# zuds-survey/zuds-pipeline

Hardware: AMD Instinct MI355X
Metric: Mpix/s resample->coadd->subtract, 3072x3072 frames (higher is better)
Workload: dtype f32; 1 GPU; configs[1]+[2]: 32x 3072x3072 TPV frames/GPU, mesh background + weight rescale + Lanczos-3 resample + WEIGHTED coadd (+ AND mask coadd, int16 masks); then 1 science frame/GPU: align ref, hotpants 3x3 regions x 10x10 stamps, r=10, ko=4, subtract; frames_per_gpu=32, size=3072, mask_dtype=int16, combine=WEIGHTED, subtract=True

## Files before the change

zuds-pipeline_amd/csrc/hotpants.hip:

```cpp
#include "hp_dev.h"
#include <sched.h>
#include "chol_diag.h"

__global__ void k_hp_valid(const float* __restrict__ sci, const float* __restrict__ ref,
                           const uint8_t* __restrict__ bpm, int64_t n, float il, float iu,
                           float tl, float tu, uint8_t* __restrict__ bad,
                           const double* __restrict__ lim, double nsig) {
    int64_t p = (int64_t)blockIdx.x * blockDim.x + threadIdx.x;
    if (lim) {
        il = (float)(lim[0] - nsig * lim[1]);
        tl = (float)(lim[3] - nsig * lim[4]);
    }
    if (p >= n) return;
    float s = sci[p], t = ref[p];
    bool ok = (s == s) && (t == t) && fabsf(s) < 3e38f && fabsf(t) < 3e38f;
    ok = ok && s >= il && s <= iu && t >= tl && t <= tu;
    if (bpm) ok = ok && bpm[p] == 0;
    bad[p] = ok ? 0 : 1;
}

#define HP_ROWMAX 16384
__global__ __launch_bounds__(256) void k_hp_rowany(const uint8_t* __restrict__ in, int nx, int ny, int hw,
                                                   uint8_t* __restrict__ out) {
    extern __shared__ int ra_pre[];
    __shared__ int wsum[4];
    const int y = blockIdx.x, tid = threadIdx.x;
    const uint8_t* row = in + (size_t)y * nx;
    const int per = (nx + 255) / 256;
    const int x0 = tid * per, x1 = min(x0 + per, nx);
    int loc = 0;
    for (int x = x0; x < x1; ++x) loc += row[x] ? 1 : 0;
    int inc = loc;
    const int lane = tid & 63, wave = tid >> 6;
#pragma unroll
    for (int o = 1; o < 64; o <<= 1) {
        const int t = __shfl_up(inc, o);
        if (lane >= o) inc += t;
    }
    if (lane == 63) wsum[wave] = inc;
    __syncthreads();
    int base = inc - loc;
    for (int w = 0; w < wave; ++w) base += wsum[w];
    if (tid == 0) ra_pre[0] = 0;
    int run = base;
    for (int x = x0; x < x1; ++x) { run += row[x] ? 1 : 0; ra_pre[x + 1] = run; }
    __syncthreads();
    for (int x = tid; x < nx; x += 256) {
        const int a = max(x - hw, 0), b = min(x + hw, nx - 1);
        out[(size_t)y * nx + x] = (ra_pre[b + 1] - ra_pre[a]) > 0;
    }
}

__global__ __launch_bounds__(256) void k_hp_valid_rows(const float* __restrict__ sci, const float* __restrict__ ref,
                                                       const uint8_t* __restrict__ bpm, int nx, int ny, float il, float iu,
                                                       float tl, float tu, const double* __restrict__ lim, double nsig,
                                                       int hw1, int hw2, uint8_t* __restrict__ bad,
                                                       uint8_t* __restrict__ out1, uint8_t* __restrict__ out2) {
    extern __shared__ int ra_pre[];
    __shared__ int wsum[HP_ROWMAX / 64], wtot[4];
    if (lim) {
        il = (float)(lim[0] - nsig * lim[1]);
        tl = (float)(lim[3] - nsig * lim[4]);
    }
    const int y = blockIdx.x, tid = threadIdx.x;
    const size_t r0 = (size_t)y * nx;
    const int lane = tid & 63, wave = tid >> 6;
    const int nch = (nx + 255) / 256;
    for (int c = 0; c < nch; ++c) {
        const int x = 256 * c + tid;
        bool b = false;
        if (x < nx) {
            const float s = sci[r0 + x], t = ref[r0 + x];
            bool ok = (s == s) && (t == t) && fabsf(s) < 3e38f && fabsf(t) < 3e38f;
            ok = ok && s >= il && s <= iu && t >= tl && t <= tu;
            if (bpm) ok = ok && bpm[r0 + x] == 0;
            b = !ok;
            bad[r0 + x] = b ? 1 : 0;
        }
        const unsigned long long m = __ballot(b);
        if (x < nx) ra_pre[x + 1] = __popcll(m & ((2ull << lane) - 1ull));
        if (lane == 0) wsum[4 * c + wave] = __popcll(m);
    }
    if (tid == 0) ra_pre[0] = 0;
    __syncthreads();
    {
        const int v = tid < 4 * nch ? wsum[tid] : 0;
        int inc = v;
#pragma unroll
        for (int o = 1; o < 64; o <<= 1) {
            const int t = __shfl_up(inc, o);
            if (lane >= o) inc += t;
        }
        if (lane == 63) wtot[wave] = inc;
        __syncthreads();
        int off = inc - v;
        for (int w = 0; w < wave; ++w) off += wtot[w];
        if (tid < 4 * nch) wsum[tid] = off;
    }
    __syncthreads();
    for (int c = 0; c < nch; ++c) {
        const int x = 256 * c + tid;
        if (x < nx) ra_pre[x + 1] += wsum[4 * c + wave];
    }
    __syncthreads();
    for (int x = tid; x < nx; x += 256) {
        const int a1 = max(x - hw1, 0), b1 = min(x + hw1, nx - 1);
        const int a2 = max(x - hw2, 0), b2 = min(x + hw2, nx - 1);
        out1[r0 + x] = (ra_pre[b1 + 1] - ra_pre[a1]) > 0;
        out2[r0 + x] = (ra_pre[b2 + 1] - ra_pre[a2]) > 0;
    }
}
// ... 387 lines not shown
        for (int k = threadIdx.x; k < nzero; k += 256) zero[(size_t)reg * nzero + k] = 0u;
    const int c1 = blockIdx.y * 16 + (threadIdx.x >> 4), c2 = blockIdx.x * 16 + (threadIdx.x & 15);
    if (blockIdx.x > blockIdx.y) return;
    if (c1 >= P.nunk || c2 >= P.nunk) return;
    int n1, p1, n2, p2;
    col_decode(P, c1, &n1, &p1);
    col_decode(P, c2, &n2, &p2);
    double acc = 0.0, racc = 0.0;
    const bool do_rhs = (c2 == 0);
    bool any = false;
    const int* list = chg + P.ncell + reg * (P.ncellr + 1);
    const int ncand = (sign == 0) ? P.ncellr : list[0];
    for (int s0 = 0; s0 < ncand; s0 += 8) {
        double g[8], gr[8], w1[8], w2[8];
        bool on[8];
#pragma unroll
        for (int u = 0; u < 8; ++u) {
            const int s = s0 + u;
            on[u] = false;
            g[u] = gr[u] = 0.0;
            w1[u] = w2[u] = 1.0;
            if (s < ncand) {
                const int cell = (sign == 0) ? reg * P.ncellr + s : list[1 + s];
                on[u] = !(active[cell] < 0 && sign >= 0);
                if (on[u]) {
                    const double* Gc = G + (size_t)cell * HP_MAXX * HP_MAXX;
                    const double* ph = phi + (size_t)cell * P.nkp;
                    if (p1 >= 0) w1[u] = ph[p1];
                    if (p2 >= 0) w2[u] = ph[p2];
                    g[u] = Gc[n1 * HP_MAXX + n2];
                    if (do_rhs) gr[u] = Gc[n1 * HP_MAXX + P.nE];
                }
            }
        }
#pragma unroll
        for (int u = 0; u < 8; ++u)
            if (on[u]) {
                any = true;
                acc += w1[u] * w2[u] * g[u];
                if (do_rhs) racc += w1[u] * gr[u];
            }
    }
    const size_t ia = (size_t)reg * (size_t)(P.nunk + 1) * P.nunk + (size_t)c1 * P.nunk + c2;
    if (sign == 0) {
        if (c2 <= c1) A[ia] = acc;
        if (do_rhs) rhs[(size_t)reg * P.nunk + c1] = racc;
    } else if (any) {
        if (c2 <= c1) A[ia] += sign * acc;
        if (do_rhs) rhs[(size_t)reg * P.nunk + c1] += sign * racc;
    }
}

#define BB_CH 128
static __device__ __forceinline__ void hp_build_blk_body(const int reg, const int pair, const hp_plan& P, const double* __restrict__ G,
                                                      const double* __restrict__ phi,
                                                      const int* __restrict__ active,
                                                      const int* __restrict__ chg, int sign,
                                                      double* __restrict__ A,
                                                      double* __restrict__ rhs, const int* __restrict__ guard,
                                                      unsigned* __restrict__ zero, int nzero,
                                                      const double* __restrict__ Gold,
                                                      const double* __restrict__ phiold,
                                                      const int* __restrict__ need) {
    if (guard && *guard == 0) return;
    int n1 = (int)((sqrtf(8.f * (float)pair + 1.f) - 1.f) * 0.5f);
    while (n1 * (n1 + 1) / 2 > pair) --n1;
    while ((n1 + 1) * (n1 + 2) / 2 <= pair) ++n1;
    const int n2 = pair - n1 * (n1 + 1) / 2;
    if (zero && n1 == 0 && n2 == 0)
        for (int k = threadIdx.x; k < nzero; k += 256) zero[(size_t)reg * nzero + k] = 0u;
    const int p1 = threadIdx.x >> 4, p2 = threadIdx.x & 15;
    const bool k1 = n1 >= 1 && n1 < P.nc, k2 = n2 >= 1 && n2 < P.nc;
    const int nk = (P.nc - 1) * P.nkp;
    const int c1 = n1 == 0 ? 0 : (k1 ? 1 + (n1 - 1) * P.nkp + p1 : 1 + nk + (n1 - P.nc));
    const int c2 = n2 == 0 ? 0 : (k2 ? 1 + (n2 - 1) * P.nkp + p2 : 1 + nk + (n2 - P.nc));
    const bool live = p1 < (k1 ? P.nkp : 1) && p2 < (k2 ? P.nkp : 1) && c2 <= c1;
    const bool do_rhs = (c2 == 0);
    const int* list = chg + P.ncell + reg * (P.ncellr + 1);
    const int ncand = (sign == 0) ? P.ncellr : list[0];
    __shared__ double gs[BB_CH], grs[BB_CH], phs[BB_CH * 16];
    __shared__ int ons[BB_CH];
    const int tid = threadIdx.x;
    const size_t ia = (size_t)reg * (size_t)(P.nunk + 1) * P.nunk + (size_t)c1 * P.nunk + c2;
    double av = 0.0, rv = 0.0;
    bool touched = false;
    const int npass = sign == 2 ? 2 : 1;
    for (int pass = 0; pass < npass; ++pass) {
        const int sg = sign == 2 ? (pass == 0 ? -1 : 1) : sign;
        double acc = 0.0, racc = 0.0;
        bool any = false;
        for (int s0 = 0; s0 < ncand; s0 += BB_CH) {
            const int nch = min(BB_CH, ncand - s0);
            __syncthreads();
            if (tid < nch) {
                const int cell = (sg == 0) ? reg * P.ncellr + s0 + tid : list[1 + s0 + tid];
                const int on = !(active[cell] < 0 && sg >= 0);
                const bool was = sign == 2 && pass == 0 && need[cell];
                const double* Gc = (was ? Gold : G) + (size_t)cell * HP_MAXX * HP_MAXX;
                ons[tid] = on;
                gs[tid] = on ? Gc[n1 * HP_MAXX + n2] : 0.0;
                grs[tid] = (on && n2 == 0) ? Gc[n1 * HP_MAXX + P.nE] : 0.0;
            }
            for (int e = tid; e < nch * P.nkp; e += 256) {
                const int k = e / P.nkp, pp = e - k * P.nkp;
                const int cell = (sg == 0) ? reg * P.ncellr + s0 + k : list[1 + s0 + k];
                const bool was = sign == 2 && pass == 0 && need[cell];
                phs[k * 16 + pp] = (was ? phiold : phi)[(size_t)cell * P.nkp + pp];
            }
            __syncthreads();
            if (live) {
                for (int k = 0; k < nch; ++k) {
                    if (!ons[k]) continue;
                    any = true;
                    const double w1 = k1 ? phs[k * 16 + p1] : 1.0, w2 = k2 ? phs[k * 16 + p2] : 1.0;
                    acc += w1 * w2 * gs[k];
                    if (do_rhs) racc += w1 * grs[k];
                }
            }
        }
        if (!live) continue;
        if (sg == 0) {
            A[ia] = acc;
            if (do_rhs) rhs[(size_t)reg * P.nunk + c1] = racc;
        } else if (any) {
            if (!touched) {
                av = A[ia];
                if (do_rhs) rv = rhs[(size_t)reg * P.nunk + c1];
                touched = true;
            }
            av += (double)sg * acc;
            if (do_rhs) rv += (double)sg * racc;
        }
    }
    if (live && touched) {
        A[ia] = av;
        if (do_rhs) rhs[(size_t)reg * P.nunk + c1] = rv;
    }
}

#define BM_CH 128
static __device__ __forceinline__ void hp_build_mfma_body(const hp_plan& P, const double* __restrict__ G,
                                                       const double* __restrict__ phi, const int* __restrict__ active,
                                                       double* __restrict__ A, double* __restrict__ rhs,
                                                       unsigned* __restrict__ zero, int nzero) {
    typedef double bm_double4 __attribute__((ext_vector_type(4)));
    __shared__ double phs[BM_CH][16];
    __shared__ double gw[4][2][BM_CH];
    const int reg = blockIdx.y, tid = threadIdx.x, wave = tid >> 6, lane = tid & 63, li = lane & 15, lk = lane >> 4;
    if (zero && blockIdx.x == 0)
        for (int k = tid; k < nzero; k += 256) zero[(size_t)reg * nzero + k] = 0u;
    const int npair = P.nE * (P.nE + 1) / 2;
    const int pair = blockIdx.x * 4 + wave;
    const bool have = pair < npair;
    int n1 = 0, n2 = 0;
    if (have) {
        n1 = (int)((sqrtf(8.f * (float)pair + 1.f) - 1.f) * 0.5f);
        while (n1 * (n1 + 1) / 2 > pair) --n1;
        while ((n1 + 1) * (n1 + 2) / 2 <= pair) ++n1;
        n2 = pair - n1 * (n1 + 1) / 2;
    }
    const bool k1 = n1 >= 1 && n1 < P.nc, k2 = n2 >= 1 && n2 < P.nc;
    const int nk = (P.nc - 1) * P.nkp;
    const int b1 = n1 == 0 ? 0 : (k1 ? 1 + (n1 - 1) * P.nkp : 1 + nk + (n1 - P.nc));
    const int b2 = n2 == 0 ? 0 : (k2 ? 1 + (n2 - 1) * P.nkp : 1 + nk + (n2 - P.nc));
    const int np1 = k1 ? P.nkp : 1, np2 = k2 ? P.nkp : 1;
    bm_double4 c4 = {0.0, 0.0, 0.0, 0.0};
    for (int s0 = 0; s0 < P.ncellr; s0 += BM_CH) {
        const int nch = min(BM_CH, P.ncellr - s0);
        __syncthreads();
        for (int e = tid; e < BM_CH * 16; e += 256) {
            const int k = e >> 4, pp = e & 15;
            double v = 0.0;
            if (k < nch && pp < P.nkp) {
                const int cell = reg * P.ncellr + s0 + k;
                if (active[cell] >= 0) v = phi[(size_t)cell * P.nkp + pp];
            }
            phs[k][pp] = v;
        }
        for (int k = lane; k < BM_CH; k += 64) {
            double g = 0.0, gr = 0.0;
            if (have && k < nch) {
                const int cell = reg * P.ncellr + s0 + k;
                if (active[cell] >= 0) {
                    const double* Gc = G + (size_t)cell * HP_MAXX * HP_MAXX;
                    g = Gc[n1 * HP_MAXX + n2];
                    if (n2 == 0) gr = Gc[n1 * HP_MAXX + P.nE];
                }
            }
            gw[wave][0][k] = g;
            gw[wave][1][k] = gr;
// ... 1428 lines not shown
    used = wave_sum_d(used);
    if (lane == 0) {
        nrej[reg] = (int)cnt;
        if (cnt > 0) atomicAdd(round_flag, (int)cnt);
        if (tmo && tmo[reg]) atomicOr(round_flag, HP_RFLAG_TMO);
        stats[reg * 2 + 0] = used > 0 ? msum / used : 0.0;
        stats[reg * 2 + 1] = used;
    }
    int* list = chg + P.ncell + reg * (P.ncellr + 1);
    int base = 0;
#pragma unroll
    for (int u = 0; u < 4; ++u) {
        const unsigned long long bm = chm[u];
        if (bm >> lane & 1ull)
            list[1 + base + __popcll(bm & ((1ull << lane) - 1ull))] = reg * P.ncellr + lane + 64 * u;
        base += __popcll(bm);
    }
    if (lane == 0) list[0] = base;
}

__global__ void k_hp_init_active(const hp_plan P, const int2* __restrict__ centres,
                                 int* __restrict__ active, int* __restrict__ need,
                                 int* __restrict__ ntotal) {
    int cell = blockIdx.x * blockDim.x + threadIdx.x;
    if (cell >= P.ncell) return;
    bool has = centres[cell * P.nss].x >= 0;
    active[cell] = has ? 0 : -1;
    need[cell] = has ? 1 : 0;
    if (has) atomicAdd(&ntotal[cell / P.ncellr], 1);
}

__global__ __launch_bounds__(256) void k_hp_gram(const hp_plan P, const double* __restrict__ X,
                                                 const int* __restrict__ need, const int* __restrict__ active,
                                                 double* __restrict__ Gp, const int* __restrict__ guard,
                                                 const int* __restrict__ list) {
    hp_gram_body(P, X, need, active, Gp, guard, list);
}
__global__ __launch_bounds__(256) void k_hp_gram_b(const hp_plan P, const hp_job* __restrict__ jobs, int round) {
    const hp_job& J = jobs[blockIdx.z];
    hp_gram_body(P, J.X, J.need, J.active, J.Gp, HPJ_GUARD(J, round), round > 1 ? J.needlist : nullptr);
}

__global__ __launch_bounds__(GS_THREADS) void k_hp_gram_sum(const double* __restrict__ Gp, const int* __restrict__ need,
                                                     const int* __restrict__ active, double* __restrict__ G,
                                                     const int* __restrict__ guard, double* __restrict__ Gold,
                                                     const int* __restrict__ list) {
    hp_gram_sum_body(Gp, need, active, G, guard, Gold, list);
}
__global__ __launch_bounds__(GS_THREADS) void k_hp_gram_sum_b(const hp_job* __restrict__ jobs, int round) {
    const hp_job& J = jobs[blockIdx.z];
    hp_gram_sum_body(J.Gp, J.need, J.active, J.G, HPJ_GUARD(J, round), J.Gold, round > 1 ? J.needlist : nullptr);
}

#define HBB_PAIRS 5
__global__ __launch_bounds__(256) void k_hp_build_blk(const hp_plan P, const double* __restrict__ G,
                                                      const double* __restrict__ phi, const int* __restrict__ active,
                                                      const int* __restrict__ chg, int sign, double* __restrict__ A,
                                                      double* __restrict__ rhs, const int* __restrict__ guard,
                                                      unsigned* __restrict__ zero = nullptr, int nzero = 0,
                                                      const double* __restrict__ Gold = nullptr,
                                                      const double* __restrict__ phiold = nullptr,
                                                      const int* __restrict__ need = nullptr) {
    if (guard && *guard == 0) return;
    const int reg = blockIdx.z;
    if (sign == 2 && chg[P.ncell + reg * (P.ncellr + 1)] == 0) {
        if (zero && blockIdx.x == 0)
            for (int k = threadIdx.x; k < nzero; k += 256) zero[(size_t)reg * nzero + k] = 0u;
        return;
    }
    const int npair = P.nE * (P.nE + 1) / 2;
#pragma unroll 1
    for (int pair = blockIdx.x * HBB_PAIRS; pair < min((int)(blockIdx.x + 1) * HBB_PAIRS, npair); ++pair)
        hp_build_blk_body(reg, pair, P, G, phi, active, chg, sign, A, rhs, guard, zero, nzero, Gold, phiold, need);
}
__global__ __launch_bounds__(256) void k_hp_build_blk_b(const hp_plan P, const hp_job* __restrict__ jobs, int round) {
    const hp_job& J = jobs[blockIdx.y];
    const int* guard = HPJ_GUARD(J, round);
    if (guard && *guard == 0) return;
    const int reg = blockIdx.z;
    if (HPJ_REGION_IDLE(J, round, reg, P.ncell, P.ncellr)) return;
    const int npair = P.nE * (P.nE + 1) / 2;
#pragma unroll 1
    for (int pair = blockIdx.x * HBB_PAIRS; pair < min((int)(blockIdx.x + 1) * HBB_PAIRS, npair); ++pair)
        hp_build_blk_body(reg, pair, P, J.G, J.phi, J.active, J.chg, round == 1 ? 0 : 2, J.A0, J.rhs0, guard,
                          nullptr, 0, J.Gold, J.phiold, J.need);
}

__global__ __launch_bounds__(256) void k_hp_build_mfma(const hp_plan P, const double* __restrict__ G,
                                                       const double* __restrict__ phi, const int* __restrict__ active,
                                                       double* __restrict__ A, double* __restrict__ rhs,
                                                       unsigned* __restrict__ zero, int nzero) {
    hp_build_mfma_body(P, G, phi, active, A, rhs, zero, nzero);
}
__global__ __launch_bounds__(256) void k_hp_build_mfma_b(const hp_plan P, const hp_job* __restrict__ jobs) {
    const hp_job& J = jobs[blockIdx.z];
    hp_build_mfma_body(P, J.G, J.phi, J.active, J.A0, J.rhs0, nullptr, 0);
}

__global__ void k_hp_diag(int n, const double* __restrict__ A, double* __restrict__ d, const int* __restrict__ guard) {
    hp_diag_body(n, A, d, guard);
}
__global__ void k_hp_diag_b(int n, const hp_job* __restrict__ jobs, int round) {
    const hp_job& J = jobs[blockIdx.z];
    hp_diag_body(n, J.A0, J.dsc, HPJ_GUARD(J, round));
}

__global__ void k_hp_scale(int n, int lda, const double* __restrict__ A0, const double* __restrict__ rhs0,
                           double* __restrict__ A, const double* __restrict__ d, unsigned* __restrict__ bar,
                           const int* __restrict__ guard, unsigned* __restrict__ dff, int ndff) {
    hp_scale_body(blockIdx.z, n, lda, A0, rhs0, A, d, bar, guard, dff, ndff);
}
#define HSB_ROWS 8
__global__ __launch_bounds__(256) void k_hp_scale_b(int n, int lda, int nreg, const hp_job* __restrict__ jobs, int round,
                                                    int ncell, int ncellr) {
    const hp_job& J = jobs[blockIdx.y / nreg];
    const int* guard = HPJ_GUARD(J, round);
    if (guard && *guard == 0) return;
    const int reg = blockIdx.y % nreg;
    if (HPJ_REGION_IDLE(J, round, reg, ncell, ncellr)) return;
    const double* __restrict__ dd = J.dsc + (size_t)reg * n;
    const double* __restrict__ A0 = J.A0 + (size_t)reg * (size_t)(n + 1) * n;
    const double* __restrict__ rhs0 = J.rhs0 + (size_t)reg * n;
    double* __restrict__ A = J.A + (size_t)reg * (size_t)(n + 1) * lda;
#pragma unroll 1
    for (int k = 0; k < HSB_ROWS; ++k) {
        const int c1 = blockIdx.x * HSB_ROWS + k;
        if (c1 >= n) break;
        const double r1 = 1.0 / dd[c1];
        for (int c2 = threadIdx.x; c2 <= c1; c2 += 256) {
            const double r2 = 1.0 / dd[c2];
            double v = __dmul_rn(A0[(size_t)c1 * n + c2], __dmul_rn(r1, r2));
            if (c1 == c2) v = __dadd_rn(v, HP_RIDGE);
            A[(size_t)c1 * lda + c2] = v;
        }
        if (threadIdx.x == 0) A[(size_t)n * lda + c1] = __dmul_rn(rhs0[c1], r1);
    }
}

// ... 147 lines not shown
        const int f = P->tfx[n];
        if (P->tfn[f] == 0) P->tf0[f] = n;
        P->tfn[f] += 1;
    }
    int nkp = 0;
    for (int i = 0; i <= P->ko; ++i)
        for (int j = 0; j <= P->ko - i; ++j) { P->kpi[nkp] = i; P->kpj[nkp] = j; ++nkp; }
    P->nkp = nkp;
    int nbg = 0;
    for (int i = 0; i <= P->bgo; ++i)
        for (int j = 0; j <= P->bgo - i; ++j) { P->bpi[nbg] = i; P->bpj[nbg] = j; ++nbg; }
    P->nbg = nbg;
    P->nE = nc + nbg;
    P->nX = P->nE + 1;
    ZM_CHECK(P->nX <= HP_MAXX, "zm_subtract: %d basis + %d background terms exceed the %d-row Gram tile", nc, nbg, HP_MAXX);
    P->nunk = 1 + (nc - 1) * nkp + nbg;
    basis->assign((size_t)nc * step * step, 0.0);
    for (int n = 0; n < nc; ++n) {
        const double* fx = filt->data() + (size_t)P->tfx[n] * step;
        const double* fy = filt->data() + (size_t)P->tfy[n] * step;
        for (int v = 0; v < step; ++v)
            for (int u = 0; u < step; ++u) {
                double k = fy[v] * fx[u] * P->tscale[n];
                if (P->tsub0[n]) k -= (*basis)[(size_t)v * step + u];
                (*basis)[((size_t)n * step + v) * step + u] = k;
            }
    }
    return 0;
}

static __device__ __forceinline__ void hp_solved_body(int nreg, int nunk, const double* __restrict__ stats, const int* __restrict__ fail,
                            const int* __restrict__ tmo, const double* __restrict__ x,
                            unsigned long long* __restrict__ mask, double* __restrict__ x0out = nullptr) {
    unsigned long long m = 0;
    const int reg = threadIdx.x;
    if (reg < nreg) {
        const double x0 = x[(size_t)reg * nunk];
        if (x0out) x0out[reg] = x0;
        const bool ok = stats[2 * reg + 1] >= 1.0 && fail[reg] == 0 && tmo[reg] == 0 && isfinite(x0);
        m = ok ? 1ull << reg : 0ull;
    }
#pragma unroll
    for (int o = 32; o >= 1; o >>= 1) m |= __shfl_xor(m, o);
    if (threadIdx.x == 0) *mask = m;
}
__global__ void k_hp_solved(int nreg, int nunk, const double* __restrict__ stats, const int* __restrict__ fail,
                            const int* __restrict__ tmo, const double* __restrict__ x,
                            unsigned long long* __restrict__ mask, double* __restrict__ x0out = nullptr) {
    hp_solved_body(nreg, nunk, stats, fail, tmo, x, mask, x0out);
}


static int hp_launch_masks(zm_ctx* ctx, const hp_plan& P, const zm_hp_params* hp, const float* sci, const float* ref,
                           const uint8_t* bpm, uint8_t* bad, uint8_t* tmp8, uint8_t* dirty, uint8_t* outbad) {
    const int nx = P.nx, ny = P.ny;
    const int64_t np = (int64_t)nx * ny;
    hipStream_t st = ctx->stream;
    const dim3 b256(256);
    zm_scope_timer t(ctx, "hp_masks");
    ZM_CHECK(nx <= HP_ROWMAX, "zm_subtract: frames wider than %d pixels are not supported", HP_ROWMAX);
    const size_t rsh = sizeof(int) * ((size_t)nx + 1);
    dim3 gc(zm_div_up(nx, 256), zm_div_up(ny, HP_COLSTRIP));
    if (!ctx->hp_rset && rsh > 65536) {
        ZM_HIP(hipFuncSetAttribute((const void*)k_hp_rowany, hipFuncAttributeMaxDynamicSharedMemorySize,
                                   (int)(sizeof(int) * (HP_ROWMAX + 1))));
        ZM_HIP(hipFuncSetAttribute((const void*)k_hp_valid_rows, hipFuncAttributeMaxDynamicSharedMemorySize,
                                   (int)(sizeof(int) * (HP_ROWMAX + 1))));
        ctx->hp_rset = true;
    }
    const bool col4 = (nx % 4 == 0) && (((uintptr_t)tmp8 | (uintptr_t)dirty | (uintptr_t)outbad) & 3) == 0;
    dim3 gc4(zm_div_up(nx / 4, 256), zm_div_up(ny, HP_COLSTRIP4));
    static const bool split = ZM_DEVENV("ZM_HP_MASKS") && !strcmp(ZM_DEVENV("ZM_HP_MASKS"), "split");
    uint8_t* tmp8b = nullptr;
    if (!split) ZM_TRY(ctx->get("hp_tmp8b", np, (void**)&tmp8b));
    if (!split && (((uintptr_t)tmp8b & 3) == 0)) {
        hipLaunchKernelGGL(k_hp_valid_rows, dim3(ny), b256, rsh, st, sci, ref, bpm, nx, ny, (float)P.il, (float)P.iu,
                           (float)P.tl, (float)P.tu, hp->limits_dev, hp->limits_nsigma, P.hw, P.hwk, bad, tmp8, tmp8b);
        if (col4) {
            hipLaunchKernelGGL(k_hp_colany4, gc4, b256, 0, st, tmp8, nx, ny, P.hw, 1, dirty);
            hipLaunchKernelGGL(k_hp_colany4, gc4, b256, 0, st, tmp8b, nx, ny, P.hwk, 1, outbad);
        } else {
            hipLaunchKernelGGL(k_hp_colany, gc, b256, 0, st, tmp8, nx, ny, P.hw, 1, dirty);
            hipLaunchKernelGGL(k_hp_colany, gc, b256, 0, st, tmp8b, nx, ny, P.hwk, 1, outbad);
        }
    } else {
        hipLaunchKernelGGL(k_hp_valid, dim3((unsigned)((np + 255) / 256)), b256, 0, st, sci, ref, bpm, np,
                           (float)P.il, (float)P.iu, (float)P.tl, (float)P.tu, bad, hp->limits_dev, hp->limits_nsigma);
        hipLaunchKernelGGL(k_hp_rowany, dim3(ny), b256, rsh, st, bad, nx, ny, P.hw, tmp8);
        if (col4) hipLaunchKernelGGL(k_hp_colany4, gc4, b256, 0, st, tmp8, nx, ny, P.hw, 1, dirty);
        else hipLaunchKernelGGL(k_hp_colany, gc, b256, 0, st, tmp8, nx, ny, P.hw, 1, dirty);
        hipLaunchKernelGGL(k_hp_rowany, dim3(ny), b256, rsh, st, bad, nx, ny, P.hwk, tmp8);
        if (col4) hipLaunchKernelGGL(k_hp_colany4, gc4, b256, 0, st, tmp8, nx, ny, P.hwk, 1, outbad);
        else hipLaunchKernelGGL(k_hp_colany, gc, b256, 0, st, tmp8, nx, ny, P.hwk, 1, outbad);
    }
    ZM_HIP(hipGetLastError());
    return 0;
}

static int hp_launch_cells(zm_ctx* ctx, const hp_plan& P, const float* ref, const uint8_t* bad, const uint8_t* dirty,
                           int2* centres, int* active, int* need, int* ntotal) {
    hipStream_t st = ctx->stream;
    const dim3 b256(256);
    zm_scope_timer t(ctx, "hp_cells");
    int maxcell = 0;
    for (int r = 0; r < P.nreg; ++r)
        maxcell = std::max(maxcell, ((P.rx1[r] - P.rx0[r]) / P.nsx) * ((P.ry1[r] - P.ry0[r]) / P.nsy));
    const char* cf = getenv("ZM_CELLS_FORM");
    if (maxcell <= HC_THREADS * HC_PX && !(cf && !strcmp(cf, "global")))
        hipLaunchKernelGGL(k_hp_cells_reg, dim3(P.ncell), dim3(HC_THREADS), 0, st, P, ref, bad, dirty, centres);
    else
        hipLaunchKernelGGL(k_hp_cells, dim3(P.ncell), b256, 0, st, P, ref, bad, dirty, centres);
    hipLaunchKernelGGL(k_hp_init_active, dim3(zm_div_up(P.ncell, 256)), b256, 0, st, P, centres, active, need, ntotal);
    ZM_HIP(hipGetLastError());
    return 0;
}

static std::atomic<int> g_hp_fitting[64];
struct hp_fit_guard {
    std::atomic<int>* c;
    int others;
    explicit hp_fit_guard(std::atomic<int>* cc) : c(cc), others(cc->fetch_add(1)) {}
    bool shared() const { return c && (others > 0 || c->load(std::memory_order_relaxed) > 1); }
    void release() { if (c) c->fetch_sub(1); c = nullptr; }
    ~hp_fit_guard() { release(); }
};

#define HP_NIBUF_ (4 * HP_MAXREG + 4)
#define HP_SUMBYTES_ (sizeof(int) * HP_NIBUF_ + sizeof(double) * 3 * HP_MAXREG)
static void hp_fill_info(const char* h_sum, int nreg, int nunk, int rounds, int retries, zm_hp_info* info) {
    const int* h_int = reinterpret_cast<const int*>(h_sum);
    const double* h_stats = reinterpret_cast<const double*>(h_sum + sizeof(int) * HP_NIBUF_);
    const double* h_x0 = h_stats + 2 * HP_MAXREG;
    auto reg_solved = [&](int reg) {
        return h_stats[2 * reg + 1] >= 1.0 && h_int[2 * HP_MAXREG + reg] == 0 &&
               h_int[3 * HP_MAXREG + 4 + reg] == 0 && std::isfinite(h_x0[reg]);
    };
    memset(info, 0, sizeof(*info));
    double ks = 0, chi = 0;
    int nsolved = 0;
    for (int r = 0; r < nreg; ++r) {
// ... 39 lines not shown
    int *active = nullptr, *need = nullptr, *ibuf = nullptr;
    double *X = nullptr, *G = nullptr, *phi = nullptr, *vbar = nullptr, *A = nullptr, *rhs = nullptr,
           *dsc = nullptr, *merit = nullptr, *stats = nullptr, *d_filt = nullptr;
    ZM_TRY(ctx->get("hp_centres", sizeof(int2) * P.ncell * P.nss, (void**)&centres));
    ZM_TRY(ctx->get("hp_active", sizeof(int) * P.ncell, (void**)&active));
    ZM_TRY(ctx->get("hp_need", sizeof(int) * P.ncell, (void**)&need));
    int* needlist = nullptr;
    ZM_TRY(ctx->get("hp_needlist", sizeof(int) * ((size_t)P.ncell + 1), (void**)&needlist));
    int* chg = nullptr;
    ZM_TRY(ctx->get("hp_chg", sizeof(int) * (2 * (size_t)P.ncell + P.nreg), (void**)&chg));
    constexpr int HP_NIBUF = 4 * HP_MAXREG + 4;
    constexpr size_t HP_SUMBYTES = sizeof(int) * HP_NIBUF + sizeof(double) * 3 * HP_MAXREG;
    static_assert((sizeof(int) * HP_NIBUF) % 8 == 0, "the statistics behind the counters are doubles");
    char* sumbuf = nullptr;
    ZM_TRY(ctx->get("hp_summary", HP_SUMBYTES, (void**)&sumbuf));
    ibuf = reinterpret_cast<int*>(sumbuf);
    int *nrej = ibuf, *ntotal = ibuf + HP_MAXREG, *fail = ibuf + 2 * HP_MAXREG, *nmasked = ibuf + 3 * HP_MAXREG;
    int* tmo = ibuf + 3 * HP_MAXREG + 4;
    unsigned* cbar = nullptr;
    ZM_TRY(ctx->get("hp_cbar", sizeof(unsigned) * CF_BAR_STRIDE * HP_MAXREG, (void**)&cbar));
    double* cdg = nullptr;
    ZM_TRY(ctx->get("hp_cdg", sizeof(double) * 4 * CH_NB * (CH_NB + 1) * HP_MAXREG, (void**)&cdg));
    ZM_TRY(ctx->get("hp_X", sizeof(double) * (size_t)P.ncell * P.nX * P.npixp, (void**)&X));
    ZM_TRY(ctx->get("hp_G", sizeof(double) * (size_t)P.ncell * HP_MAXX * HP_MAXX, (void**)&G));
    double* Gp = nullptr;
    ZM_TRY(ctx->get("hp_Gp", sizeof(double) * (size_t)P.ncell * GR_SPLIT * HP_MAXX * HP_MAXX, (void**)&Gp));
    ZM_TRY(ctx->get("hp_phi", sizeof(double) * (size_t)P.ncell * P.nkp, (void**)&phi));
    double *Gold = nullptr, *phiold = nullptr;
    ZM_TRY(ctx->get("hp_Gold", sizeof(double) * (size_t)P.ncell * HP_MAXX * HP_MAXX, (void**)&Gold));
    ZM_TRY(ctx->get("hp_phiold", sizeof(double) * (size_t)P.ncell * P.nkp, (void**)&phiold));
    ZM_TRY(ctx->get("hp_vbar", sizeof(double) * P.ncell, (void**)&vbar));
    const int lda = (P.nunk + 15) & ~15;
    ZM_TRY(ctx->get("hp_A", sizeof(double) * (size_t)P.nreg * (P.nunk + 1) * lda, (void**)&A));
    ZM_TRY(ctx->get("hp_rhs", sizeof(double) * (size_t)P.nreg * P.nunk, (void**)&rhs));
    double *A0 = nullptr, *rhs0 = nullptr;
    ZM_TRY(ctx->get("hp_A0", sizeof(double) * (size_t)P.nreg * (P.nunk + 1) * P.nunk, (void**)&A0));
    ZM_TRY(ctx->get("hp_rhs0", sizeof(double) * (size_t)P.nreg * P.nunk, (void**)&rhs0));
    ZM_TRY(ctx->get("hp_dsc", sizeof(double) * (size_t)P.nreg * P.nunk, (void**)&dsc));
    ZM_TRY(ctx->get("hp_merit", sizeof(double) * P.ncell, (void**)&merit));
    stats = reinterpret_cast<double*>(sumbuf + sizeof(int) * HP_NIBUF);
    double* x0sum = stats + 2 * HP_MAXREG;
    ZM_TRY(ctx->get("hp_filt", sizeof(double) * filt.size(), (void**)&d_filt));
    if (!(ctx->hp_filt_dev == (const void*)d_filt && ctx->hp_filt_host == filt)) {
        double* h_tab = nullptr;
        ZM_TRY(ctx->get_pinned("hp_tab", sizeof(double) * filt.size(), (void**)&h_tab));
        ZM_HIP(hipStreamSynchronize(st));
        memcpy(h_tab, filt.data(), sizeof(double) * filt.size());
        ZM_HIP(hipMemcpyAsync(d_filt, h_tab, sizeof(double) * filt.size(), hipMemcpyHostToDevice, st));
        ctx->hp_filt_host = filt;
        ctx->hp_filt_dev = d_filt;
    }

    const dim3 b256(256);
    ZM_TRY(hp_launch_masks(ctx, P, hp, sci, ref, bpm, bad, tmp8, dirty, outbad));
    char* h_sum = nullptr;
    ZM_TRY(ctx->get_pinned("hp_summary_h", HP_SUMBYTES, (void**)&h_sum));
    const int* h_int = reinterpret_cast<const int*>(h_sum);
    const double* h_stats = reinterpret_cast<const double*>(h_sum + sizeof(int) * HP_NIBUF);
    const double* h_x0 = h_stats + 2 * HP_MAXREG;
    int rounds = 0, retries = 0, ntimeouts = 0;
    const char* spin_env = getenv("ZM_CHOL_SPIN_LIMIT");
    hp_fit_guard fitting(&g_hp_fitting[ctx->device & 63]);
    for (int attempt = 0; attempt < 2; ++attempt) {
    const bool safe = attempt > 0;
    const int spin_limit = (!safe && spin_env) ? atoi(spin_env) : CF_SPIN_LIMIT;
    ZM_HIP(hipMemsetAsync(ibuf, 0, sizeof(int) * HP_NIBUF, st));
    ZM_TRY(hp_launch_cells(ctx, P, ref, bad, dirty, centres, active, need, ntotal));
    const hv_cfg hvc = hp_vectors_cfg(P.pw, P.sw, P.npix);
    ZM_CHECK(hvc.cw >= 8, "zm_subtract: r = %d, rss = %d: the template patch alone exceeds the LDS", P.hwk, P.hwss);
    size_t vsh = hvc.shmem;
    const int hv_gx = hvc.big ? std::min(P.ncell, 128) : P.ncell;
    double* hv_w0g = nullptr;
    if (hvc.w0_global)
        ZM_TRY(ctx->get("hp_w0g", sizeof(double) * (size_t)hv_gx * HV_SPLIT_FEW * P.npix, (void**)&hv_w0g));

    int* rflags = nullptr;
    int* h_rflags = nullptr;
    hipEvent_t* evs = nullptr;
    ZM_TRY(ctx->get("hp_rflags", sizeof(int) * 32, (void**)&rflags));
    ZM_TRY(ctx->get_pinned("hp_rflags_h", sizeof(int) * 16, (void**)&h_rflags));
    ZM_TRY(zm_get_sync_events(ctx, 3, &evs));
    ZM_HIP(hipMemsetAsync(rflags, 0, sizeof(int) * 32, st));
    if (!ctx->hp_sig_h) {
        ZM_HIP(hipHostMalloc((void**)&ctx->hp_sig_h, sizeof(unsigned long long) * 16, hipHostMallocCoherent | hipHostMallocMapped));
        memset(ctx->hp_sig_h, 0, sizeof(unsigned long long) * 16);
        ZM_HIP(hipHostGetDevicePointer((void**)&ctx->hp_sig_d, ctx->hp_sig_h, 0));
    }
    static const bool sig_off = ZM_DEVENV("ZM_HP_SIGNAL") && ZM_DEVENV("ZM_HP_SIGNAL")[0] == '0';
    const unsigned seq = ++ctx->hp_seq;
    auto enqueue_round = [&](const int rounds) -> int {
        const int* guard = rounds > 1 ? rflags + (rounds - 1) : nullptr;
        const int ncl_grid = std::min(P.ncell, 48);
        if (rounds > 1) {
            zm_scope_timer t(ctx, "hp_solve");
            int nt = zm_div_up(P.nunk, 16);
            if (P.nkp > 16)
                hipLaunchKernelGGL(k_hp_build, dim3(nt, nt, P.nreg), b256, 0, st, P, G, phi, active, chg, -1, A0, rhs0, guard);
        }
        {
            zm_scope_timer t(ctx, "hp_vectors");
            ZM_TRY(zm_hp_launch_vectors(ctx, st, P, hvc, rounds, ncl_grid, hv_gx, sci, ref, sci_rms, ref_rms, d_filt, centres, active,
                                        need, X, phi, vbar, guard, phiold, needlist, hv_w0g));
            ZM_HIP(hipGetLastError());
        }
        {
            zm_scope_timer t(ctx, "hp_gram");
            hipLaunchKernelGGL(k_hp_gram, dim3(rounds == 1 ? P.ncell : ncl_grid, GR_SPLIT), b256, 0, st, P, X, need, active, Gp, guard,
                               rounds == 1 ? nullptr : needlist);
            hipLaunchKernelGGL(k_hp_gram_sum, dim3(rounds == 1 ? P.ncell : ncl_grid), dim3(GS_THREADS), 0, st, Gp, need, active, G, guard, Gold,
                               rounds == 1 ? nullptr : needlist);
            ZM_HIP(hipGetLastError());
        }
        {
            zm_scope_timer t(ctx, "hp_solve");
            int nt = zm_div_up(P.nunk, 16);
            const char* form_env = getenv("ZM_CHOL_FORM");
            bool tp = safe || ctx->share >= 2 || fitting.shared();
            if (form_env && !strcmp(form_env, "tp")) tp = true;
            if (form_env && (!strcmp(form_env, "lat") || !strcmp(form_env, "df")) && !safe) tp = false;
            if (!ctx->hp_wg_cap) {
                int occ = 0, ncu = 0;
                ZM_HIP(hipOccupancyMaxActiveBlocksPerMultiprocessor(&occ, (const void*)k_chol_fused, 256, 0));
                ZM_HIP(hipDeviceGetAttribute(&ncu, hipDeviceAttributeMultiprocessorCount, ctx->device));
                ctx->hp_wg_cap = std::max(1, std::min(occ, 1) * (ncu - ncu / 16));
                if (ZM_DEVENV("ZM_CHOL_PROF")) fprintf(stderr, "chol: occupancy %d x %d CUs\n", occ, ncu);
            }
            const int wg_cap = ctx->hp_wg_cap / std::max(ctx->share, 1);
            const int W = std::max(2, std::min(68, wg_cap / P.nreg));
            const int nunk = P.nunk;
            static const bool want_prof = ZM_DEVENV("ZM_CHOL_PROF") && atoi(ZM_DEVENV("ZM_CHOL_PROF")) != 0;
            const bool want_df = !tp && !(form_env && !strcmp(form_env, "lat")) && 2 * P.nreg <= wg_cap && W <= 128;
            const int ndff = hp_df_nflags(P.nunk);
            unsigned* dff = nullptr;
            double* dfdg = nullptr;
            int* dftiles = nullptr;
// ... 560 lines not shown
```

Baseline: 49430 Mpix/s.

## Fold ibuf/rflags zeroing into mask kernel and batch normal-matrix update over pairs

Two memsets on the first attempt are replaced by zeroing work inside block 0 of the validity/mask kernel, which removes two small stream operations. The sign==2 incremental normal-matrix update is rewritten as its own body. That body handles five Gram pairs per block in one pass over the changed-cell list, loading old and new G/phi into shared memory once and accumulating the subtract and add-back terms together rather than running two separate passes per pair. This adds register pressure from the per-pair arrays, and the early-exit idle-region check in the batched kernel is now replaced by the ncand<=0 return.

```diff
diff --git a/zuds-pipeline_amd/csrc/hotpants.hip b/zuds-pipeline_amd/csrc/hotpants.hip
--- a/zuds-pipeline_amd/csrc/hotpants.hip
+++ b/zuds-pipeline_amd/csrc/hotpants.hip
@@ -2,11 +2,19 @@
 #include <sched.h>
 #include "chol_diag.h"
 
+static __device__ __forceinline__ void hp_zero_words(int* __restrict__ zero0, int nzero0, int* __restrict__ zero1, int nzero1) {
+    if (blockIdx.x != 0) return;
+    if (zero0) for (int k = threadIdx.x; k < nzero0; k += blockDim.x) zero0[k] = 0;
+    if (zero1) for (int k = threadIdx.x; k < nzero1; k += blockDim.x) zero1[k] = 0;
+}
 __global__ void k_hp_valid(const float* __restrict__ sci, const float* __restrict__ ref,
                            const uint8_t* __restrict__ bpm, int64_t n, float il, float iu,
                            float tl, float tu, uint8_t* __restrict__ bad,
-                           const double* __restrict__ lim, double nsig) {
+                           const double* __restrict__ lim, double nsig,
+                           int* __restrict__ zero0 = nullptr, int nzero0 = 0,
+                           int* __restrict__ zero1 = nullptr, int nzero1 = 0) {
     int64_t p = (int64_t)blockIdx.x * blockDim.x + threadIdx.x;
+    hp_zero_words(zero0, nzero0, zero1, nzero1);
     if (lim) {
         il = (float)(lim[0] - nsig * lim[1]);
         tl = (float)(lim[3] - nsig * lim[4]);
@@ -55,8 +63,11 @@
                                                        const uint8_t* __restrict__ bpm, int nx, int ny, float il, float iu,
                                                        float tl, float tu, const double* __restrict__ lim, double nsig,
                                                        int hw1, int hw2, uint8_t* __restrict__ bad,
-                                                       uint8_t* __restrict__ out1, uint8_t* __restrict__ out2) {
+                                                       uint8_t* __restrict__ out1, uint8_t* __restrict__ out2,
+                                                       int* __restrict__ zero0 = nullptr, int nzero0 = 0,
+                                                       int* __restrict__ zero1 = nullptr, int nzero1 = 0) {
     extern __shared__ int ra_pre[];
+    hp_zero_words(zero0, nzero0, zero1, nzero1);
     __shared__ int wsum[HP_ROWMAX / 64], wtot[4];
     if (lim) {
         il = (float)(lim[0] - nsig * lim[1]);
@@ -550,21 +561,29 @@
 }
 
 #define BB_CH 128
+#define HBB_PAIRS 5
+#define BU_CH 32
+#define BB_LDS (BB_CH * 18 + BB_CH / 2)
+static __device__ __forceinline__ void hp_pair_decode(const int pair, int* n1o, int* n2o) {
+    int n1 = (int)((sqrtf(8.f * (float)pair + 1.f) - 1.f) * 0.5f);
+    while (n1 * (n1 + 1) / 2 > pair) --n1;
+    while ((n1 + 1) * (n1 + 2) / 2 <= pair) ++n1;
+    *n1o = n1;
+    *n2o = pair - n1 * (n1 + 1) / 2;
+}
+static __device__ __forceinline__ void hp_blk_entry_add(const double w1, const double w2, const double g, const double gr,
+                                                     const bool do_rhs, double& acc, double& racc) {
+    acc += w1 * w2 * g;
+    if (do_rhs) racc += w1 * gr;
+}
 static __device__ __forceinline__ void hp_build_blk_body(const int reg, const int pair, const hp_plan& P, const double* __restrict__ G,
                                                       const double* __restrict__ phi,
                                                       const int* __restrict__ active,
-                                                      const int* __restrict__ chg, int sign,
                                                       double* __restrict__ A,
-                                                      double* __restrict__ rhs, const int* __restrict__ guard,
-                                                      unsigned* __restrict__ zero, int nzero,
-                                                      const double* __restrict__ Gold,
-                                                      const double* __restrict__ phiold,
-                                                      const int* __restrict__ need) {
-    if (guard && *guard == 0) return;
-    int n1 = (int)((sqrtf(8.f * (float)pair + 1.f) - 1.f) * 0.5f);
-    while (n1 * (n1 + 1) / 2 > pair) --n1;
-    while ((n1 + 1) * (n1 + 2) / 2 <= pair) ++n1;
-    const int n2 = pair - n1 * (n1 + 1) / 2;
+                                                      double* __restrict__ rhs,
+                                                      unsigned* __restrict__ zero, int nzero, double* sh) {
+    int n1, n2;
+    hp_pair_decode(pair, &n1, &n2);
     if (zero && n1 == 0 && n2 == 0)
         for (int k = threadIdx.x; k < nzero; k += 256) zero[(size_t)reg * nzero + k] = 0u;
     const int p1 = threadIdx.x >> 4, p2 = threadIdx.x & 15;
@@ -574,66 +593,161 @@
     const int c2 = n2 == 0 ? 0 : (k2 ? 1 + (n2 - 1) * P.nkp + p2 : 1 + nk + (n2 - P.nc));
     const bool live = p1 < (k1 ? P.nkp : 1) && p2 < (k2 ? P.nkp : 1) && c2 <= c1;
     const bool do_rhs = (c2 == 0);
-    const int* list = chg + P.ncell + reg * (P.ncellr + 1);
-    const int ncand = (sign == 0) ? P.ncellr : list[0];
-    __shared__ double gs[BB_CH], grs[BB_CH], phs[BB_CH * 16];
-    __shared__ int ons[BB_CH];
+    double *gs = sh, *grs = sh + BB_CH, *phs = sh + 2 * BB_CH;
+    int* ons = reinterpret_cast<int*>(sh + 18 * BB_CH);
     const int tid = threadIdx.x;
     const size_t ia = (size_t)reg * (size_t)(P.nunk + 1) * P.nunk + (size_t)c1 * P.nunk + c2;
-    double av = 0.0, rv = 0.0;
-    bool touched = false;
-    const int npass = sign == 2 ? 2 : 1;
-    for (int pass = 0; pass < npass; ++pass) {
-        const int sg = sign == 2 ? (pass == 0 ? -1 : 1) : sign;
-        double acc = 0.0, racc = 0.0;
-        bool any = false;
-        for (int s0 = 0; s0 < ncand; s0 += BB_CH) {
-            const int nch = min(BB_CH, ncand - s0);
-            __syncthreads();
-            if (tid < nch) {
-                const int cell = (sg == 0) ? reg * P.ncellr + s0 + tid : list[1 + s0 + tid];
-                const int on = !(active[cell] < 0 && sg >= 0);
-                const bool was = sign == 2 && pass == 0 && need[cell];
-                const double* Gc = (was ? Gold : G) + (size_t)cell * HP_MAXX * HP_MAXX;
-                ons[tid] = on;
-                gs[tid] = on ? Gc[n1 * HP_MAXX + n2] : 0.0;
-                grs[tid] = (on && n2 == 0) ? Gc[n1 * HP_MAXX + P.nE] : 0.0;
-            }
-            for (int e = tid; e < nch * P.nkp; e += 256) {
-                const int k = e / P.nkp, pp = e - k * P.nkp;
-                const int cell = (sg == 0) ? reg * P.ncellr + s0 + k : list[1 + s0 + k];
-                const bool was = sign == 2 && pass == 0 && need[cell];
-                phs[k * 16 + pp] = (was ? phiold : phi)[(size_t)cell * P.nkp + pp];
-            }
-            __syncthreads();
-            if (live) {
-                for (int k = 0; k < nch; ++k) {
-                    if (!ons[k]) continue;
-                    any = true;
-                    const double w1 = k1 ? phs[k * 16 + p1] : 1.0, w2 = k2 ? phs[k * 16 + p2] : 1.0;
-                    acc += w1 * w2 * gs[k];
-                    if (do_rhs) racc += w1 * grs[k];
-                }
-            }
-        }
-        if (!live) continue;
-        if (sg == 0) {
-            A[ia] = acc;
-            if (do_rhs) rhs[(size_t)reg * P.nunk + c1] = racc;
-        } else if (any) {
-            if (!touched) {
-                av = A[ia];
-                if (do_rhs) rv = rhs[(size_t)reg * P.nunk + c1];
-                touched = true;
-            }
-            av += (double)sg * acc;
-            if (do_rhs) rv += (double)sg * racc;
-        }
-    }
-    if (live && touched) {
-        A[ia] = av;
-        if (do_rhs) rhs[(size_t)reg * P.nunk + c1] = rv;
-    }
+    double acc = 0.0, racc = 0.0;
+    for (int s0 = 0; s0 < P.ncellr; s0 += BB_CH) {
+        const int nch = min(BB_CH, P.ncellr - s0);
+        __syncthreads();
+        if (tid < nch) {
+            const int cell = reg * P.ncellr + s0 + tid;
+            const int on = active[cell] >= 0;
+            const double* Gc = G + (size_t)cell * HP_MAXX * HP_MAXX;
+            ons[tid] = on;
+            gs[tid] = on ? Gc[n1 * HP_MAXX + n2] : 0.0;
+            grs[tid] = (on && n2 == 0) ? Gc[n1 * HP_MAXX + P.nE] : 0.0;
+        }
+        for (int e = tid; e < nch * P.nkp; e += 256) {
+            const int k = e / P.nkp, pp = e - k * P.nkp;
+            phs[k * 16 + pp] = phi[(size_t)(reg * P.ncellr + s0 + k) * P.nkp + pp];
+        }
+        __syncthreads();
+        if (live) {
+            for (int k = 0; k < nch; ++k) {
+                if (!ons[k]) continue;
+                const double w1 = k1 ? phs[k * 16 + p1] : 1.0, w2 = k2 ? phs[k * 16 + p2] : 1.0;
+                hp_blk_entry_add(w1, w2, gs[k], do_rhs ? grs[k] : 0.0, do_rhs, acc, racc);
+            }
+        }
+    }
+    if (!live) return;
+    A[ia] = acc;
+    if (do_rhs) rhs[(size_t)reg * P.nunk + c1] = racc;
+}
+
+static __device__ __forceinline__ void hp_update_blk_body(const int reg, const int pair0, const hp_plan& P, const double* __restrict__ G,
+                                                       const double* __restrict__ phi, const int* __restrict__ active,
+                                                       const int* __restrict__ chg, double* __restrict__ A,
+                                                       double* __restrict__ rhs, unsigned* __restrict__ zero, int nzero,
+                                                       const double* __restrict__ Gold, const double* __restrict__ phiold,
+                                                       const int* __restrict__ need, double* sh) {
+    static_assert(HBB_PAIRS * BU_CH <= 256 && BU_CH * 16 == 512, "one Gram item and two spatial-term items per thread");
+    static_assert(4 * HBB_PAIRS * BU_CH + 2 * BU_CH * 16 + BU_CH <= BB_LDS, "the update's staging fits the build's LDS");
+    double (*ug)[HBB_PAIRS][BU_CH] = reinterpret_cast<double (*)[HBB_PAIRS][BU_CH]>(sh);
+    double (*ugr)[HBB_PAIRS][BU_CH] = reinterpret_cast<double (*)[HBB_PAIRS][BU_CH]>(sh + 2 * HBB_PAIRS * BU_CH);
+    double (*uph)[BU_CH * 16] = reinterpret_cast<double (*)[BU_CH * 16]>(sh + 4 * HBB_PAIRS * BU_CH);
+    int* uon = reinterpret_cast<int*>(sh + 4 * HBB_PAIRS * BU_CH + 2 * BU_CH * 16);
+    const int tid = threadIdx.x;
+    const int npair = P.nE * (P.nE + 1) / 2;
+    if (zero && pair0 == 0)
+        for (int k = tid; k < nzero; k += 256) zero[(size_t)reg * nzero + k] = 0u;
+    const int* list = chg + P.ncell + reg * (P.ncellr + 1);
+    const int ncand = list[0];
+    if (ncand <= 0) return;
+    const int p1 = tid >> 4, p2 = tid & 15;
+    const int nk = (P.nc - 1) * P.nkp;
+    bool k1[HBB_PAIRS], k2[HBB_PAIRS], live[HBB_PAIRS], do_rhs[HBB_PAIRS], any1[HBB_PAIRS];
+    size_t ia[HBB_PAIRS], ir[HBB_PAIRS];
+    double av[HBB_PAIRS], rv[HBB_PAIRS], acc0[HBB_PAIRS], racc0[HBB_PAIRS], acc1[HBB_PAIRS], racc1[HBB_PAIRS];
+    {
+        int n1, n2;
+        hp_pair_decode(pair0, &n1, &n2);
+#pragma unroll
+        for (int q = 0; q < HBB_PAIRS; ++q) {
+            k1[q] = n1 >= 1 && n1 < P.nc;
+            k2[q] = n2 >= 1 && n2 < P.nc;
+            const int c1 = n1 == 0 ? 0 : (k1[q] ? 1 + (n1 - 1) * P.nkp + p1 : 1 + nk + (n1 - P.nc));
+            const int c2 = n2 == 0 ? 0 : (k2[q] ? 1 + (n2 - 1) * P.nkp + p2 : 1 + nk + (n2 - P.nc));
+            live[q] = pair0 + q < npair && p1 < (k1[q] ? P.nkp : 1) && p2 < (k2[q] ? P.nkp : 1) && c2 <= c1;
+            do_rhs[q] = (c2 == 0);
+            ia[q] = (size_t)reg * (size_t)(P.nunk + 1) * P.nunk + (size_t)c1 * P.nunk + c2;
+            ir[q] = (size_t)reg * P.nunk + c1;
+            any1[q] = false;
+            av[q] = rv[q] = acc0[q] = racc0[q] = acc1[q] = racc1[q] = 0.0;
+            if (live[q]) {
+                av[q] = A[ia[q]];
+                if (do_rhs[q]) rv[q] = rhs[ir[q]];
+            }
+            if (++n2 > n1) { ++n1; n2 = 0; }
+        }
+    }
+    const int gq = min(tid / BU_CH, HBB_PAIRS - 1), gk = tid % BU_CH;
+    const bool gdo = tid < HBB_PAIRS * BU_CH && pair0 + gq < npair;
+    int gn1, gn2;
+    hp_pair_decode(min(pair0 + gq, npair - 1), &gn1, &gn2);
+    for (int s0 = 0; s0 < ncand; s0 += BU_CH) {
+        const int nch = min(BU_CH, ncand - s0);
+        __syncthreads();
+        {
+            const int cg = list[1 + s0 + min(gk, nch - 1)];
+            int cp[2], pp[2];
+#pragma unroll
+            for (int u = 0; u < 2; ++u) {
+                const int e = tid + 256 * u;
+                cp[u] = list[1 + s0 + min(e >> 4, nch - 1)];
+                pp[u] = min(e & 15, P.nkp - 1);
+            }
+            const int wasg = need[cg], ong = active[cg] >= 0;
+            const double* Gn = G + (size_t)cg * HP_MAXX * HP_MAXX;
+            const double* Go = Gold + (size_t)cg * HP_MAXX * HP_MAXX;
+            const double gnew = Gn[gn1 * HP_MAXX + gn2], gold = Go[gn1 * HP_MAXX + gn2];
+            const double rnew = Gn[gn1 * HP_MAXX + P.nE], rold = Go[gn1 * HP_MAXX + P.nE];
+            int wasp[2];
+            double fnew[2], fold[2];
+#pragma unroll
+            for (int u = 0; u < 2; ++u) {
+                wasp[u] = need[cp[u]];
+                fnew[u] = phi[(size_t)cp[u] * P.nkp + pp[u]];
+                fold[u] = phiold[(size_t)cp[u] * P.nkp + pp[u]];
+            }
+            if (gdo && gk < nch) {
+                ug[0][gq][gk] = wasg ? gold : gnew;
+                ugr[0][gq][gk] = gn2 == 0 ? (wasg ? rold : rnew) : 0.0;
+                ug[1][gq][gk] = ong ? gnew : 0.0;
+                ugr[1][gq][gk] = (ong && gn2 == 0) ? rnew : 0.0;
+                if (gq == 0) uon[gk] = ong;
+            }
+#pragma unroll
+            for (int u = 0; u < 2; ++u) {
+                const int e = tid + 256 * u;
+                if ((e >> 4) < nch && (e & 15) < P.nkp) {
+                    uph[0][e] = wasp[u] ? fold[u] : fnew[u];
+                    uph[1][e] = fnew[u];
+                }
+            }
+        }
+        __syncthreads();
+        for (int k = 0; k < nch; ++k) {
+            const double f1o = uph[0][k * 16 + p1], f2o = uph[0][k * 16 + p2];
+            const double f1n = uph[1][k * 16 + p1], f2n = uph[1][k * 16 + p2];
+            const bool back = uon[k] != 0;
+#pragma unroll
+            for (int q = 0; q < HBB_PAIRS; ++q)
+                if (live[q]) {
+                    hp_blk_entry_add(k1[q] ? f1o : 1.0, k2[q] ? f2o : 1.0, ug[0][q][k], do_rhs[q] ? ugr[0][q][k] : 0.0,
+                                     do_rhs[q], acc0[q], racc0[q]);
+                    if (back) {
+                        any1[q] = true;
+                        hp_blk_entry_add(k1[q] ? f1n : 1.0, k2[q] ? f2n : 1.0, ug[1][q][k], do_rhs[q] ? ugr[1][q][k] : 0.0,
+                                         do_rhs[q], acc1[q], racc1[q]);
+                    }
+                }
+        }
+    }
+#pragma unroll
+    for (int q = 0; q < HBB_PAIRS; ++q)
+        if (live[q]) {
+            av[q] += -1.0 * acc0[q];
+            if (do_rhs[q]) rv[q] += -1.0 * racc0[q];
+            if (any1[q]) {
+                av[q] += acc1[q];
+                if (do_rhs[q]) rv[q] += racc1[q];
+            }
+            A[ia[q]] = av[q];
+            if (do_rhs[q]) rhs[ir[q]] = rv[q];
+        }
 }
 
 #define BM_CH 128
@@ -2168,7 +2282,6 @@
     hp_gram_sum_body(J.Gp, J.need, J.active, J.G, HPJ_GUARD(J, round), J.Gold, round > 1 ? J.needlist : nullptr);
 }
 
-#define HBB_PAIRS 5
 __global__ __launch_bounds__(256) void k_hp_build_blk(const hp_plan P, const double* __restrict__ G,
                                                       const double* __restrict__ phi, const int* __restrict__ active,
                                                       const int* __restrict__ chg, int sign, double* __restrict__ A,
@@ -2177,29 +2290,33 @@
                                                       const double* __restrict__ Gold = nullptr,
                                                       const double* __restrict__ phiold = nullptr,
                                                       const int* __restrict__ need = nullptr) {
+    __shared__ double sh[BB_LDS];
     if (guard && *guard == 0) return;
     const int reg = blockIdx.z;
-    if (sign == 2 && chg[P.ncell + reg * (P.ncellr + 1)] == 0) {
-        if (zero && blockIdx.x == 0)
-            for (int k = threadIdx.x; k < nzero; k += 256) zero[(size_t)reg * nzero + k] = 0u;
+    if (sign == 2) {
+        hp_update_blk_body(reg, blockIdx.x * HBB_PAIRS, P, G, phi, active, chg, A, rhs, zero, nzero, Gold, phiold, need, sh);
         return;
     }
     const int npair = P.nE * (P.nE + 1) / 2;
 #pragma unroll 1
     for (int pair = blockIdx.x * HBB_PAIRS; pair < min((int)(blockIdx.x + 1) * HBB_PAIRS, npair); ++pair)
-        hp_build_blk_body(reg, pair, P, G, phi, active, chg, sign, A, rhs, guard, zero, nzero, Gold, phiold, need);
+        hp_build_blk_body(reg, pair, P, G, phi, active, A, rhs, zero, nzero, sh);
 }
 __global__ __launch_bounds__(256) void k_hp_build_blk_b(const hp_plan P, const hp_job* __restrict__ jobs, int round) {
+    __shared__ double sh[BB_LDS];
     const hp_job& J = jobs[blockIdx.y];
     const int* guard = HPJ_GUARD(J, round);
     if (guard && *guard == 0) return;
     const int reg = blockIdx.z;
-    if (HPJ_REGION_IDLE(J, round, reg, P.ncell, P.ncellr)) return;
+    if (round > 1) {
+        hp_update_blk_body(reg, blockIdx.x * HBB_PAIRS, P, J.G, J.phi, J.active, J.chg, J.A0, J.rhs0, nullptr, 0, J.Gold,
+                           J.phiold, J.need, sh);
+        return;
+    }
     const int npair = P.nE * (P.nE + 1) / 2;
 #pragma unroll 1
     for (int pair = blockIdx.x * HBB_PAIRS; pair < min((int)(blockIdx.x + 1) * HBB_PAIRS, npair); ++pair)
-        hp_build_blk_body(reg, pair, P, J.G, J.phi, J.active, J.chg, round == 1 ? 0 : 2, J.A0, J.rhs0, guard,
-                          nullptr, 0, J.Gold, J.phiold, J.need);
+        hp_build_blk_body(reg, pair, P, J.G, J.phi, J.active, J.A0, J.rhs0, nullptr, 0, sh);
 }
 
 __global__ __launch_bounds__(256) void k_hp_build_mfma(const hp_plan P, const double* __restrict__ G,
@@ -2453,7 +2570,8 @@
 
 
 static int hp_launch_masks(zm_ctx* ctx, const hp_plan& P, const zm_hp_params* hp, const float* sci, const float* ref,
-                           const uint8_t* bpm, uint8_t* bad, uint8_t* tmp8, uint8_t* dirty, uint8_t* outbad) {
+                           const uint8_t* bpm, uint8_t* bad, uint8_t* tmp8, uint8_t* dirty, uint8_t* outbad,
+                           int* zero0 = nullptr, int nzero0 = 0, int* zero1 = nullptr, int nzero1 = 0) {
     const int nx = P.nx, ny = P.ny;
     const int64_t np = (int64_t)nx * ny;
     hipStream_t st = ctx->stream;
@@ -2476,7 +2594,8 @@
     if (!split) ZM_TRY(ctx->get("hp_tmp8b", np, (void**)&tmp8b));
     if (!split && (((uintptr_t)tmp8b & 3) == 0)) {
         hipLaunchKernelGGL(k_hp_valid_rows, dim3(ny), b256, rsh, st, sci, ref, bpm, nx, ny, (float)P.il, (float)P.iu,
-                           (float)P.tl, (float)P.tu, hp->limits_dev, hp->limits_nsigma, P.hw, P.hwk, bad, tmp8, tmp8b);
+                           (float)P.tl, (float)P.tu, hp->limits_dev, hp->limits_nsigma, P.hw, P.hwk, bad, tmp8, tmp8b, zero0, nzero0,
+                           zero1, nzero1);
         if (col4) {
             hipLaunchKernelGGL(k_hp_colany4, gc4, b256, 0, st, tmp8, nx, ny, P.hw, 1, dirty);
             hipLaunchKernelGGL(k_hp_colany4, gc4, b256, 0, st, tmp8b, nx, ny, P.hwk, 1, outbad);
@@ -2486,7 +2605,8 @@
         }
     } else {
         hipLaunchKernelGGL(k_hp_valid, dim3((unsigned)((np + 255) / 256)), b256, 0, st, sci, ref, bpm, np,
-                           (float)P.il, (float)P.iu, (float)P.tl, (float)P.tu, bad, hp->limits_dev, hp->limits_nsigma);
+                           (float)P.il, (float)P.iu, (float)P.tl, (float)P.tu, bad, hp->limits_dev, hp->limits_nsigma, zero0, nzero0,
+                           zero1, nzero1);
         hipLaunchKernelGGL(k_hp_rowany, dim3(ny), b256, rsh, st, bad, nx, ny, P.hw, tmp8);
         if (col4) hipLaunchKernelGGL(k_hp_colany4, gc4, b256, 0, st, tmp8, nx, ny, P.hw, 1, dirty);
         else hipLaunchKernelGGL(k_hp_colany, gc, b256, 0, st, tmp8, nx, ny, P.hw, 1, dirty);
@@ -2632,7 +2752,9 @@
     }
 
     const dim3 b256(256);
-    ZM_TRY(hp_launch_masks(ctx, P, hp, sci, ref, bpm, bad, tmp8, dirty, outbad));
+    int* rflags = nullptr;
+    ZM_TRY(ctx->get("hp_rflags", sizeof(int) * 32, (void**)&rflags));
+    ZM_TRY(hp_launch_masks(ctx, P, hp, sci, ref, bpm, bad, tmp8, dirty, outbad, ibuf, HP_NIBUF, rflags, 32));
     char* h_sum = nullptr;
     ZM_TRY(ctx->get_pinned("hp_summary_h", HP_SUMBYTES, (void**)&h_sum));
     const int* h_int = reinterpret_cast<const int*>(h_sum);
@@ -2644,7 +2766,7 @@
     for (int attempt = 0; attempt < 2; ++attempt) {
     const bool safe = attempt > 0;
     const int spin_limit = (!safe && spin_env) ? atoi(spin_env) : CF_SPIN_LIMIT;
-    ZM_HIP(hipMemsetAsync(ibuf, 0, sizeof(int) * HP_NIBUF, st));
+    if (attempt > 0) ZM_HIP(hipMemsetAsync(ibuf, 0, sizeof(int) * HP_NIBUF, st));
     ZM_TRY(hp_launch_cells(ctx, P, ref, bad, dirty, centres, active, need, ntotal));
     const hv_cfg hvc = hp_vectors_cfg(P.pw, P.sw, P.npix);
     ZM_CHECK(hvc.cw >= 8, "zm_subtract: r = %d, rss = %d: the template patch alone exceeds the LDS", P.hwk, P.hwss);
@@ -2654,13 +2776,11 @@
     if (hvc.w0_global)
         ZM_TRY(ctx->get("hp_w0g", sizeof(double) * (size_t)hv_gx * HV_SPLIT_FEW * P.npix, (void**)&hv_w0g));
 
-    int* rflags = nullptr;
     int* h_rflags = nullptr;
     hipEvent_t* evs = nullptr;
-    ZM_TRY(ctx->get("hp_rflags", sizeof(int) * 32, (void**)&rflags));
     ZM_TRY(ctx->get_pinned("hp_rflags_h", sizeof(int) * 16, (void**)&h_rflags));
     ZM_TRY(zm_get_sync_events(ctx, 3, &evs));
-    ZM_HIP(hipMemsetAsync(rflags, 0, sizeof(int) * 32, st));
+    if (attempt > 0) ZM_HIP(hipMemsetAsync(rflags, 0, sizeof(int) * 32, st));
     if (!ctx->hp_sig_h) {
         ZM_HIP(hipHostMalloc((void**)&ctx->hp_sig_h, sizeof(unsigned long long) * 16, hipHostMallocCoherent | hipHostMallocMapped));
         memset(ctx->hp_sig_h, 0, sizeof(unsigned long long) * 16);
```

After: 50070 Mpix/s, median of 6. 1.01x the previous value.
